# KadAMRN/Data_Free_Quantization

Hardware: AMD Instinct MI355X
Metric: weight-GB/s quantized (per-ch INT8 DFQ sweep) + top-1 delta, MobileNetV2 (higher is better)
Workload: dtype f32

## Files before the change

data_free_quantization_amd/csrc/dfq_common.h:

```cpp
#pragma once
#include <hip/hip_runtime.h>
#include <stdint.h>
#include <stdlib.h>
#include "dfq_hip.h"
#include "dfq_cle_plan.h"

namespace dfq {

__device__ __forceinline__ uint32_t enc_ord(float f) {
    uint32_t u = __float_as_uint(f);
    return (u & 0x80000000u) ? ~u : (u | 0x80000000u);
}
__device__ __forceinline__ float dec_ord(uint32_t e) {
    uint32_t u = (e & 0x80000000u) ? (e & 0x7fffffffu) : ~e;
    return __uint_as_float(u);
}

__device__ __forceinline__ float dpp_f(float v, int ctrl) {
    const int x = __float_as_int(v);
    switch (ctrl) {
        case 0xB1: return __int_as_float(__builtin_amdgcn_update_dpp(x, x, 0xB1, 0xF, 0xF, false));
        case 0x4E: return __int_as_float(__builtin_amdgcn_update_dpp(x, x, 0x4E, 0xF, 0xF, false));
        case 0x141: return __int_as_float(__builtin_amdgcn_update_dpp(x, x, 0x141, 0xF, 0xF, false));
        default: return __int_as_float(__builtin_amdgcn_update_dpp(x, x, 0x140, 0xF, 0xF, false));
// ... 331 lines not shown
__device__ inline float wave_full_sum(Get get, int64_t n, int threads, int lane, float* slots) {
    int64_t nt = 1;
    if (n >= 32768 && threads > 1) nt = ceil_div(n, (int64_t)32768) < threads ? ceil_div(n, (int64_t)32768) : threads;
    if (nt == 1) return wave_inner_sum(get, n, lane);
    const int64_t chunk = ceil_div(n, nt);
    for (int t = lane; t < threads; t += 64) slots[t] = 0.f;
    wave_lds_sync();
    for (int64_t t = 0; t < nt && t * chunk < n; ++t) {
        const int64_t b0 = t * chunk, len = (b0 + chunk < n ? b0 + chunk : n) - b0;
        const float s = wave_inner_sum([&](int64_t i) { return get(b0 + i); }, len, lane);
        if (lane == 0) slots[t] = s;
    }
    wave_lds_sync();
    float r = 0.f;
    if (lane == 0) r = aten_inner_sum([&](int64_t t) { return slots[t]; }, (int64_t)threads);
    wave_lds_sync();
    return __shfl(r, 0, 64);
}

#define DFQ_GLOBAL __attribute__((address_space(1)))
#define DFQ_LDS __attribute__((address_space(3)))
typedef float f32x4 __attribute__((ext_vector_type(4)));

__device__ __forceinline__ void st_coh(float* p, float v) {
    __hip_atomic_store(reinterpret_cast<uint32_t*>(p), __float_as_uint(v), __ATOMIC_RELAXED,
                       __HIP_MEMORY_SCOPE_AGENT);
}
__device__ __forceinline__ float ld_coh(const float* p) {
    return __uint_as_float(__hip_atomic_load(reinterpret_cast<const uint32_t*>(p), __ATOMIC_RELAXED,
                                             __HIP_MEMORY_SCOPE_AGENT));
}
__device__ __forceinline__ float ld_coh(const DFQ_GLOBAL float* p) {
    return __uint_as_float(__hip_atomic_load((const DFQ_GLOBAL uint32_t*)p, __ATOMIC_RELAXED,
                                             __HIP_MEMORY_SCOPE_AGENT));
}

__host__ __device__ inline bool aten_outer_col_is_cascade(int64_t R, int64_t F, int64_t c, int threads) {
    int64_t c0 = 0, c1 = F;
    if (R * F >= 32768 && threads > 1) {
        const int64_t nt = F < threads ? F : threads;
        const int64_t chunk = ceil_div(F, nt);
        c0 = c1 = -1;
        for (int64_t t = 0; t < nt; ++t) {
            int64_t b = t * chunk, e = b + chunk < F ? b + chunk : F;
            if (b >= F) break;
            b = b >= F ? b : b - b % 32;
            e = e >= F ? e : e - e % 32;
            if (b <= c && c < e) { c0 = b; c1 = e; break; }
        }
        if (c0 < 0) { c0 = 0; c1 = F; }
    }
    const int64_t w = c1 - c0;
    const int64_t g = w >= 8 ? 32 : 4;
    return (c - c0) < g * (w / g);
}

__host__ __device__ inline float aten_outer_col_sum(const float* a, int64_t R, int64_t F, int64_t c, int threads) {
    int64_t c0 = 0, c1 = F;
    if (R * F >= 32768 && threads > 1) {
        const int64_t nt = F < threads ? F : threads;
        const int64_t chunk = ceil_div(F, nt);
        c0 = c1 = -1;
        for (int64_t t = 0; t < nt; ++t) {
            int64_t b = t * chunk, e = b + chunk < F ? b + chunk : F;
            if (b >= F) break;
            b = b >= F ? b : b - b % 32;
            e = e >= F ? e : e - e % 32;
            if (b <= c && c < e) { c0 = b; c1 = e; break; }
        }
        if (c0 < 0) { c0 = 0; c1 = F; }
    }
    const int64_t w = c1 - c0;
    const int64_t g = w >= 8 ? 32 : 4;
    const bool cascade = (c - c0) < g * (w / g);
    auto get = [&](int64_t r) { return a[r * F + c]; };
    return cascade ? aten_cascade(get, R) : aten_row_sum(get, R);
}

}

namespace dfq {
void set_last_hip_error(hipError_t e);
void set_last_hip_error_text(const char* msg);
hipError_t stage_h2d(void* dst, const void* src, size_t bytes, hipStream_t s);
}
#define DFQ_HIP_CHECK(expr)                                   \
    do {                                                      \
        hipError_t _e = (expr);                               \
        if (_e != hipSuccess) {                               \
            dfq::set_last_hip_error(_e);                      \
            return DFQ_ERR_HIP;                               \
        }                                                     \
    } while (0)
#define DFQ_LAUNCH_CHECK()                                    \
    do {                                                      \
        hipError_t _e = hipGetLastError();                    \
        if (_e != hipSuccess) {                               \
            dfq::set_last_hip_error(_e);                      \
            return DFQ_ERR_HIP;                               \
        }                                                     \
    } while (0)
```

data_free_quantization_amd/csrc/dfq_lib.hip:

```cpp
#include "dfq_common.h"

#include <algorithm>
#include <cstring>
#include <mutex>
#include <vector>

namespace dfq {
static thread_local char g_last_hip[256] = "";
void set_last_hip_error(hipError_t e) {
    const char* msg = hipGetErrorString(e);
    size_t i = 0;
    for (; msg && msg[i] && i + 1 < sizeof(g_last_hip); ++i) g_last_hip[i] = msg[i];
    g_last_hip[i] = '\0';
}
void set_last_hip_error_text(const char* msg) {
    size_t i = 0;
    for (; msg && msg[i] && i + 1 < sizeof(g_last_hip); ++i) g_last_hip[i] = msg[i];
    g_last_hip[i] = '\0';
}

namespace {
struct StageSlot {
    void* host = nullptr;
    size_t cap = 0;
    hipEvent_t ev = nullptr;
    int device = -1;
    uint64_t last_use = 0;
};
constexpr size_t kStageMinBytes = 1 << 20;
constexpr size_t kStageMaxSlots = 32;
std::mutex g_stage_mu;
std::vector<StageSlot> g_stage;
uint64_t g_stage_tick = 0;
}

hipError_t stage_h2d(void* dst, const void* src, size_t bytes, hipStream_t s) {
    if (bytes == 0) return hipSuccess;
    int dev = 0;
    hipError_t e = hipStreamGetDevice(s, &dev);
    if (e != hipSuccess) return e;
    std::lock_guard<std::mutex> lock(g_stage_mu);
    StageSlot* slot = nullptr;
    StageSlot* oldest = nullptr;
    size_t on_dev = 0;
    for (auto& sl : g_stage) {
        if (sl.device != dev) continue;
        ++on_dev;
        if (sl.cap >= bytes && hipEventQuery(sl.ev) == hipSuccess &&
            (!slot || sl.cap < slot->cap)) slot = &sl;
        if (!oldest || sl.last_use < oldest->last_use) oldest = &sl;
    }
    if (!slot && on_dev >= kStageMaxSlots && oldest) {
        if ((e = hipEventSynchronize(oldest->ev)) != hipSuccess) return e;
        if (oldest->cap < bytes) {
            (void)hipHostFree(oldest->host);
            oldest->host = nullptr;
            oldest->cap = 0;
            size_t cap = std::max(bytes, kStageMinBytes);
            if ((e = hipHostMalloc(&oldest->host, cap, hipHostMallocDefault)) != hipSuccess) return e;
            oldest->cap = cap;
        }
        slot = oldest;
    }
    if (!slot) {
        StageSlot ns;
        ns.device = dev;
        ns.cap = std::max(bytes, kStageMinBytes);
        int cur = 0;
        if ((e = hipGetDevice(&cur)) != hipSuccess) return e;
        if (cur != dev && (e = hipSetDevice(dev)) != hipSuccess) return e;
        e = hipHostMalloc(&ns.host, ns.cap, hipHostMallocDefault);
        if (e == hipSuccess) e = hipEventCreateWithFlags(&ns.ev, hipEventDisableTiming);
        if (cur != dev) (void)hipSetDevice(cur);
        if (e != hipSuccess) {
            if (ns.host) (void)hipHostFree(ns.host);
            return e;
        }
        g_stage.push_back(ns);
        slot = &g_stage.back();
    }
    std::memcpy(slot->host, src, bytes);
    if ((e = hipMemcpyAsync(dst, slot->host, bytes, hipMemcpyHostToDevice, s)) != hipSuccess) return e;
    slot->last_use = ++g_stage_tick;
    return hipEventRecord(slot->ev, s);
}
}

namespace dfq {
static hipError_t stage_preload(size_t n) {
    int dev = 0;
    hipError_t e = hipGetDevice(&dev);
    if (e != hipSuccess) return e;
    std::lock_guard<std::mutex> lock(g_stage_mu);
    size_t on_dev = 0;
    for (const auto& sl : g_stage) on_dev += sl.device == dev ? 1 : 0;
    for (; on_dev < n && on_dev < kStageMaxSlots; ++on_dev) {
        StageSlot ns;
        ns.device = dev;
        ns.cap = kStageMinBytes;
        if ((e = hipHostMalloc(&ns.host, ns.cap, hipHostMallocDefault)) != hipSuccess) return e;
        if ((e = hipEventCreateWithFlags(&ns.ev, hipEventDisableTiming)) != hipSuccess) {
            (void)hipHostFree(ns.host);
            return e;
        }
        g_stage.push_back(ns);
    }
    return hipSuccess;
}
constexpr size_t kStagePreloadSlots = 8;

hipError_t preload_sweep();
hipError_t preload_transform();
hipError_t preload_cle();
hipError_t preload_stats();
hipError_t preload_clip();
hipError_t preload_mx();
}

extern "C" int dfq_preload(void) {
    DFQ_HIP_CHECK(dfq::preload_sweep());
    DFQ_HIP_CHECK(dfq::preload_transform());
    DFQ_HIP_CHECK(dfq::preload_cle());
    DFQ_HIP_CHECK(dfq::preload_stats());
    DFQ_HIP_CHECK(dfq::preload_clip());
    DFQ_HIP_CHECK(dfq::preload_mx());
    DFQ_HIP_CHECK(dfq::stage_preload(dfq::kStagePreloadSlots));
    return DFQ_OK;
}

extern "C" int dfq_abi_version(void) { return DFQ_ABI_VERSION; }

extern "C" const char* dfq_last_hip_error(void) { return dfq::g_last_hip; }

extern "C" const char* dfq_error_string(int code) {
    switch (code) {
        case DFQ_OK: return "ok";
        case DFQ_ERR_INVALID: return "invalid argument";
        case DFQ_ERR_HIP: return "HIP runtime error";
        case DFQ_ERR_UNSUPPORTED: return "unsupported request";
        case DFQ_ERR_NOMEM: return "out of memory";
        case DFQ_ERR_SHAPE: return "shape mismatch";
        case DFQ_ERR_WORKSPACE: return "workspace too small";
        default: return "unknown error";
    }
}
```

data_free_quantization_amd/csrc/dfq_transform.hip:

```cpp
#include "dfq_common.h"

#include <cstdlib>
#include <cstring>

#include <algorithm>
#include <chrono>
#include <cmath>
#include <mutex>
#include <new>
#include <string>
#include <vector>

namespace dfq {

static int blocks_for(int64_t n, int per_thread = 1) {
    const int64_t b = ceil_div(std::max<int64_t>(n, 1), (int64_t)kThreads * per_thread);
    return (int)std::min<int64_t>(b, 256 * 8);
}

__device__ __forceinline__ float bn_factor(float g, float v, float eps) {
    return g / sqrtf(v + eps);
}

__global__ void bn_fold_weight_kernel(float* __restrict__ w, const float* __restrict__ g,
                                      const float* __restrict__ v, float eps, int64_t rows, int64_t len) {
    const int64_t n = rows * len;
    for (int64_t i = (int64_t)blockIdx.x * blockDim.x + threadIdx.x; i < n; i += (int64_t)gridDim.x * blockDim.x) {
        const int64_t o = i / len;
        w[i] = w[i] * bn_factor(g[o], v[o], eps);
    }
}

__global__ void bn_fold_channel_kernel(float* __restrict__ bias, float* __restrict__ g, float* __restrict__ b,
                                       float* __restrict__ m, float* __restrict__ v, float* __restrict__ fake_w,
                                       float* __restrict__ fake_b, float eps, int64_t rows) {
    for (int64_t o = (int64_t)blockIdx.x * blockDim.x + threadIdx.x; o < rows; o += (int64_t)gridDim.x * blockDim.x) {
        const float go = g[o], bo = b[o], mo = m[o], vo = v[o];
        const float f = bn_factor(go, vo, eps);
        const float shift = bo - (go * mo) / sqrtf(vo + eps);
        bias[o] = bias[o] * f + shift;
        if (fake_w) fake_w[o] = fabsf(go);
        if (fake_b) fake_b[o] = bo;
        g[o] = 1.0f;
        v[o] = 1.0f;
        b[o] = 0.0f;
        m[o] = 0.0f;
    }
}

__global__ void clamp_kernel(float* __restrict__ w, int64_t n, float lo, float hi) {
    const int64_t n4 = n >> 2;
    float4* w4 = reinterpret_cast<float4*>(w);
    for (int64_t i = (int64_t)blockIdx.x * blockDim.x + threadIdx.x; i < n4; i += (int64_t)gridDim.x * blockDim.x) {
        float4 v = w4[i];
        v.x = fminf(fmaxf(v.x, lo), hi);
        v.y = fminf(fmaxf(v.y, lo), hi);
        v.z = fminf(fmaxf(v.z, lo), hi);
        v.w = fminf(fmaxf(v.w, lo), hi);
        w4[i] = v;
    }
    for (int64_t i = 4 * n4 + (int64_t)blockIdx.x * blockDim.x + threadIdx.x; i < n; i += (int64_t)gridDim.x * blockDim.x)
        w[i] = fminf(fmaxf(w[i], lo), hi);
}

__device__ __forceinline__ float absorb_c(float beta, float gamma, float n_sigma) {
    float c = beta - n_sigma * gamma;
    return (c < 0.0f) ? 0.0f : c;
}

__global__ void absorb_gemv_kernel(const float* __restrict__ w2, float* __restrict__ b2,
                                   const float* __restrict__ bn_w, const float* __restrict__ bn_b,
                                   int64_t o2, int64_t i2, int64_t khw2, int64_t o2g, float n_sigma) {
    const int lane = threadIdx.x & 63;
    const int64_t wave = (int64_t)blockIdx.x * (blockDim.x / 64) + (threadIdx.x >> 6);
    const int64_t nwaves = (int64_t)gridDim.x * (blockDim.x / 64);
    for (int64_t o = wave; o < o2; o += nwaves) {
        const int64_t g = o / o2g;
        const float* row = w2 + o * i2 * khw2;
        float acc = 0.f;
        for (int64_t i = lane; i < i2; i += 64) {
            float ssum = 0.f;
            for (int64_t k = 0; k < khw2; ++k) ssum += row[i * khw2 + k];
            const int64_t ch = g * i2 + i;
// ... 172 lines not shown
            const float x0 = (-b) / w;
            const float P0 = std_pdf(x0), C0 = std_cdf(x0);
            m = w * P0 + b * (1.0f - C0);
            const float B = ((b * b + w * w) + m * m) - (2.0f * m) * b;
            v = ((1.0f - C0) * B + (w * (b - 2.0f * m)) * P0) + (m * m) * C0;
        } else {
            const float x0 = (-b) / w, x6 = (6.0f - b) / w;
            const float P0 = std_pdf(x0), C0 = std_cdf(x0), P6 = std_pdf(x6), C6 = std_cdf(x6);
            m = (w * (P0 - P6) + b * (C6 - C0)) + 6.0f * (1.0f - C6);
            const float B = ((b * b + w * w) + m * m) - (2.0f * m) * b;
            const float d6 = 6.0f - m;
            v = ((((C6 - C0) * B + (w * -6.0f) * P6) + (w * (b - 2.0f * m)) * (P0 - P6)) + (m * m) * C0) +
                (d6 * d6) * (1.0f - C6);
        }
        if (accumulate) {
            m = mean[j] + m;
            v = var[j] + v;
        }
        mean[j] = m;
        var[j] = v;
    }
}

__global__ void act_minmax_kernel(const float* a, const float* w_in, int64_t n, int w_is_var, float eps, float nsig,
                                  float* out) {
    __shared__ float smin[4], smax[4];
    float vmin = INFINITY, vmax = -INFINITY;
    for (int64_t j = threadIdx.x; j < n; j += blockDim.x) {
        const float w = w_is_var ? sqrtf(w_in[j] + eps) : w_in[j];
        const float nw = nsig * w;
        vmin = fminf(vmin, a[j] - nw);
        vmax = fmaxf(vmax, a[j] + nw);
    }
    vmin = wave_min(vmin);
    vmax = wave_max(vmax);
    if ((threadIdx.x & 63) == 0) {
        smin[threadIdx.x >> 6] = vmin;
        smax[threadIdx.x >> 6] = vmax;
    }
    __syncthreads();
    if (threadIdx.x == 0) {
        for (int k = 1; k < (int)(blockDim.x / 64); ++k) {
            vmin = fminf(vmin, smin[k]);
            vmax = fmaxf(vmax, smax[k]);
        }
        out[0] = fminf(smin[0], vmin);
        out[1] = fmaxf(smax[0], vmax);
    }
}

__global__ void act_affine_kernel(const float* x, const float* w, const float* bias, int64_t o, int64_t i2,
                                  int64_t khw, int64_t og, float* out) {
    const int lane = threadIdx.x & 63;
    const int64_t wave = (int64_t)blockIdx.x * (blockDim.x / 64) + (threadIdx.x >> 6);
    const int64_t nwaves = (int64_t)gridDim.x * (blockDim.x / 64);
    for (int64_t r = wave; r < o; r += nwaves) {
        const int64_t g = r / og;
        float acc = 0.f;
        for (int64_t i = lane; i < i2; i += 64) {
            const float* p = w + (r * i2 + i) * khw;
            const float ws = khw == 1 ? p[0] : aten_inner_sum([&](int64_t k) { return p[k]; }, khw);
            acc += ws * x[g * i2 + i];
        }
        acc = wave_sum_f(acc);
        if (lane == 0) out[r] = bias ? acc + bias[r] : acc;
    }
}


struct BnFoldJob {
    float* w;
    float* bias;
    float* g;
    float* b;
    float* m;
    float* v;
    float* fake_w;
    float* fake_b;
    float eps;
    int32_t flags;
    int64_t rows, row_len;
    uint32_t* range_enc;
};
struct BnFoldChunk {
    int32_t job;
    int32_t pad;
    int64_t e0, e1;
};

__device__ __forceinline__ float fold_factor(const BnFoldJob& J, int64_t o) {
    const float go = ((const DFQ_GLOBAL float*)J.g)[o], ve = ((const DFQ_GLOBAL float*)J.v)[o] + J.eps;
    return (go == 1.0f && ve == 1.0f) ? 1.0f : go / sqrtf(ve);
}

__device__ __forceinline__ int64_t fold_row(const BnFoldJob& J, int64_t r0, int64_t base, float inv, int64_t i,
                                            int* rem_out) {
    const int li = (int)(i - base);
    const int len = (int)J.row_len;
    int q = (int)((float)li * inv);
    int rem = li - q * len;
    if (rem < 0) {
        --q;
        rem += len;
    } else if (rem >= len) {
        ++q;
        rem -= len;
    }
    *rem_out = rem;
    return r0 + q;
}

__device__ __forceinline__ float fold_one(const BnFoldJob& J, int64_t r0, int64_t base, float inv, int64_t i,
                                          float w) {
    int rem;
    const float f = fold_factor(J, fold_row(J, r0, base, inv, i, &rem));
    return f != 1.0f ? w * f : w;
}

__global__ void __launch_bounds__(kThreads)
bn_fold_weight_batch_kernel(const BnFoldJob* __restrict__ jobs, const BnFoldChunk* __restrict__ chunks,
                            int64_t nchunks) {
    __shared__ float smn[kThreads / kWave], smx[kThreads / kWave];
    for (int64_t c = blockIdx.x; c < nchunks; c += gridDim.x) {
        const BnFoldChunk ch = chunks[c];
        const BnFoldJob J = jobs[ch.job];
        const int64_t r0 = ch.e0 / J.row_len, base = r0 * J.row_len;
        const float inv = 1.0f / (float)J.row_len;
        float a = INFINITY, b = -INFINITY;
        const int64_t n = ch.e1 - ch.e0;
        int64_t done = 0;
        int ident = 1;
        for (int64_t r = r0 + threadIdx.x; r <= (ch.e1 - 1) / J.row_len; r += blockDim.x)
            ident &= fold_factor(J, r) == 1.0f;
        ident = __syncthreads_and(ident);
        if (ident && (reinterpret_cast<uintptr_t>(J.w + ch.e0) & 15) == 0) {
            const DFQ_GLOBAL f32x4* w4 = (const DFQ_GLOBAL f32x4*)(J.w + ch.e0);
            const int64_t n4 = n >> 2;
            for (int64_t k = threadIdx.x; k < n4; k += 4 * (int64_t)blockDim.x) {
                f32x4 v[4];
#pragma unroll
                for (int u = 0; u < 4; ++u)
                    if (k + u * (int64_t)blockDim.x < n4) v[u] = w4[k + u * blockDim.x];
#pragma unroll
                for (int u = 0; u < 4; ++u)
                    if (k + u * (int64_t)blockDim.x < n4) {
                        a = fminf(a, fminf(fminf(v[u].x, v[u].y), fminf(v[u].z, v[u].w)));
                        b = fmaxf(b, fmaxf(fmaxf(v[u].x, v[u].y), fmaxf(v[u].z, v[u].w)));
                    }
            }
            done = 4 * n4;
        } else if ((reinterpret_cast<uintptr_t>(J.w + ch.e0) & 15) == 0) {
            DFQ_GLOBAL f32x4* w4 = (DFQ_GLOBAL f32x4*)(J.w + ch.e0);
            const int64_t n4 = n >> 2;
            for (int64_t k = threadIdx.x; k < n4; k += blockDim.x) {
                const f32x4 v = w4[k];
                const int64_t i = ch.e0 + 4 * k;
                f32x4 o;
                int rem;
                const float f = fold_factor(J, fold_row(J, r0, base, inv, i, &rem));
                if (rem + 3 < (int)J.row_len) {
                    o.x = f != 1.0f ? v.x * f : v.x;
                    o.y = f != 1.0f ? v.y * f : v.y;
                    o.z = f != 1.0f ? v.z * f : v.z;
                    o.w = f != 1.0f ? v.w * f : v.w;
                } else {
                    o.x = f != 1.0f ? v.x * f : v.x;
                    o.y = fold_one(J, r0, base, inv, i + 1, v.y);
                    o.z = fold_one(J, r0, base, inv, i + 2, v.z);
                    o.w = fold_one(J, r0, base, inv, i + 3, v.w);
                }
                if (__float_as_uint(o.x) != __float_as_uint(v.x) || __float_as_uint(o.y) != __float_as_uint(v.y) ||
                    __float_as_uint(o.z) != __float_as_uint(v.z) || __float_as_uint(o.w) != __float_as_uint(v.w))
                    w4[k] = o;
                a = fminf(a, fminf(fminf(o.x, o.y), fminf(o.z, o.w)));
                b = fmaxf(b, fmaxf(fmaxf(o.x, o.y), fmaxf(o.z, o.w)));
            }
            done = 4 * n4;
        }
        DFQ_GLOBAL float* wg = (DFQ_GLOBAL float*)J.w;
        for (int64_t k = done + threadIdx.x; k < n; k += blockDim.x) {
            const int64_t i = ch.e0 + k;
            const float v = wg[i];
            const float o = fold_one(J, r0, base, inv, i, v);
            if (__float_as_uint(o) != __float_as_uint(v)) wg[i] = o;
            a = fminf(a, o);
            b = fmaxf(b, o);
        }
        if (J.range_enc) {
            a = wave_min(a);
            b = wave_max(b);
            const int lane = threadIdx.x & (kWave - 1), wv = threadIdx.x >> 6;
            if (lane == 0) {
                smn[wv] = a;
                smx[wv] = b;
            }
            __syncthreads();
            if (threadIdx.x == 0) {
                for (int k = 1; k < kThreads / kWave; ++k) {
                    a = fminf(a, smn[k]);
                    b = fmaxf(b, smx[k]);
                }
                atomicMax(&J.range_enc[0], ~enc_ord(a));
                atomicMax(&J.range_enc[1], enc_ord(b));
            }
            __syncthreads();
        }
    }
}

__global__ void bn_fold_channel_batch_kernel(const BnFoldJob* __restrict__ jobs, int32_t njobs) {
    for (int32_t j = blockIdx.x; j < njobs; j += gridDim.x) {
        const BnFoldJob J = jobs[j];
        typedef DFQ_GLOBAL float* G;
        const G g = (G)J.g, b = (G)J.b, m = (G)J.m, v = (G)J.v, bias = (G)J.bias, fw = (G)J.fake_w, fb = (G)J.fake_b;
        for (int64_t o = threadIdx.x; o < J.rows; o += blockDim.x) {
            const float go = g[o], bo = b[o], mo = m[o], vo = v[o];
            const float f = bn_factor(go, vo, J.eps);
            const float shift = bo - (go * mo) / sqrtf(vo + J.eps);
            const float b0 = (J.flags & DFQ_BN_FOLD_ZERO_BIAS) ? 0.0f : bias[o];
            bias[o] = b0 * f + shift;
            if (J.fake_w) fw[o] = fabsf(go);
            if (J.fake_b) fb[o] = bo;
            g[o] = 1.0f;
            v[o] = 1.0f;
            b[o] = 0.0f;
            m[o] = 0.0f;
        }
    }
}

__device__ __forceinline__ float qdq_nan(float x, const QParams& p, float& q) {
    const float y = qdq(x, p, q);
    return x != x ? x : y;
}

__global__ void __launch_bounds__(kThreads)
fq_given_kernel(const float* __restrict__ x, float* __restrict__ y, int64_t n, int bits, int sym, int flags,
                const float* __restrict__ min_dev, const float* __restrict__ max_dev,
                const uint32_t* __restrict__ range_enc, double gmin, double gmax, int vec4) {
    if (min_dev) gmin = (double)min_dev[0];
    if (max_dev) gmax = (double)max_dev[0];
    if (range_enc) {
        gmin = (double)dec_ord(~range_enc[0]);
        gmax = (double)dec_ord(range_enc[1]);
    }
    const QParams p = make_qparams((float)gmin, (float)gmax, bits, sym != 0, flags | DFQ_GIVEN_RANGE, gmin, gmax);
    const int64_t stride = (int64_t)gridDim.x * blockDim.x;
    float q;
    if (vec4) {
        const int64_t n4 = n >> 2;
        for (int64_t i = (int64_t)blockIdx.x * blockDim.x + threadIdx.x; i < n4; i += stride) {
            const float4 v = reinterpret_cast<const float4*>(x)[i];
            float4 o;
            o.x = qdq_nan(v.x, p, q);
            o.y = qdq_nan(v.y, p, q);
            o.z = qdq_nan(v.z, p, q);
            o.w = qdq_nan(v.w, p, q);
            reinterpret_cast<float4*>(y)[i] = o;
        }
    } else {
        for (int64_t i = (int64_t)blockIdx.x * blockDim.x + threadIdx.x; i < n; i += stride)
            y[i] = qdq_nan(x[i], p, q);
    }
}

constexpr int64_t kFqSmall = 16384;

__global__ void __launch_bounds__(kThreads)
fq_tensor_small_kernel(const float* __restrict__ x, float* __restrict__ y, int64_t n, int bits, int sym, int flags) {
    __shared__ float smn[kThreads / kWave], smx[kThreads / kWave];
    float a = INFINITY, b = -INFINITY;
    for (int64_t i = threadIdx.x; i < n; i += kThreads) {
        const float v = x[i];
        a = fminf(a, v);
        b = fmaxf(b, v);
    }
    a = wave_min(a);
    b = wave_max(b);
    const int lane = threadIdx.x & (kWave - 1), w = threadIdx.x >> 6;
    if (lane == 0) {
        smn[w] = a;
        smx[w] = b;
    }
    __syncthreads();
    for (int k = 0; k < kThreads / kWave; ++k) {
        a = k ? fminf(a, smn[k]) : smn[0];
        b = k ? fmaxf(b, smx[k]) : smx[0];
    }
// ... 640 lines not shown
    for (int32_t k = 0; k < n_ops; ++k) {
        const dfq_bc_op& op = ops[k];
        int rc = DFQ_OK;
        if (op.kind == DFQ_BC_OP_EXPECT) {
            dfq::BcLayerJob J{};
            const int32_t used = dfq::bc_layer_group(ops, n_ops, k, J);
            if (used > 0) {
                const int64_t pb = J.fake_b ? std::min<int64_t>(ceil_div(J.F, (int64_t)4), 2048) : 0;
                hipLaunchKernelGGL(dfq::bc_layer_kernel, dim3((int)(J.apply_blocks + pb)), dim3(kThreads), 0,
                                   static_cast<hipStream_t>(stream), J);
                const hipError_t e = hipGetLastError();
                if (e != hipSuccess) {
                    dfq::set_last_hip_error(e);
                    return fail(k, DFQ_ERR_HIP);
                }
                k += used - 1;
                continue;
            }
        }
        if (op.kind == DFQ_BC_OP_COPY) {
            CopyBatch b{};
            int cnt = 0;
            int64_t most = 0;
            int32_t j = k;
            for (; j < n_ops && ops[j].kind == DFQ_BC_OP_COPY && cnt < kCopyBatch; ++j) {
                if (ops[j].n == 0) continue;
                b.src[cnt] = ops[j].a;
                b.dst[cnt] = ops[j].out;
                b.n[cnt] = ops[j].n;
                most = std::max(most, ops[j].n);
                ++cnt;
            }
            if (cnt > 0) {
                hipLaunchKernelGGL(copy_batch_kernel, dim3(blocks_for(most), cnt), dim3(256), 0,
                                   static_cast<hipStream_t>(stream), b);
                const hipError_t e = hipGetLastError();
                if (e != hipSuccess) {
                    dfq::set_last_hip_error(e);
                    return fail(k, DFQ_ERR_HIP);
                }
            }
            k = j - 1;
            continue;
        }
        if (op.kind == DFQ_BC_OP_EXPECT)
            rc = dfq_bc_expect(op.a, op.b, op.n, op.flag & 1, (op.flag >> 1) & 1, op.out, stream);
        else if (op.kind == DFQ_BC_OP_APPLY)
            rc = dfq_bc_apply(op.a, op.n, op.i2, op.b, op.f, op.out, op.out2, nullptr, stream);
        else
            rc = dfq_bc_propagate(op.a, op.n, op.out, op.f, op.flag, stream);
        if (rc != DFQ_OK) return fail(k, rc);
    }
    return DFQ_OK;
}

extern "C" int dfq_act_moments(const float* w, const float* b, int64_t n, int32_t kind, int32_t sqrt_w, float eps,
                               int32_t accumulate, float* mean, float* var, void* stream) {
    if (!w || !b || !mean || !var || n < 0 || kind < 0 || kind > 2) return DFQ_ERR_INVALID;
    if (n == 0) return DFQ_OK;
    hipLaunchKernelGGL(act_moments_kernel, dim3(blocks_for(n)), dim3(kThreads), 0, static_cast<hipStream_t>(stream), w,
                       b, n, (int)kind, (int)sqrt_w, eps, (int)accumulate, mean, var);
    DFQ_LAUNCH_CHECK();
    return DFQ_OK;
}

extern "C" int dfq_act_minmax(const float* a, const float* w, int64_t n, int32_t w_is_var, float eps, float nsig,
                              float* out2, void* stream) {
    if (!a || !w || !out2 || n <= 0) return DFQ_ERR_INVALID;
    hipLaunchKernelGGL(act_minmax_kernel, dim3(1), dim3(kThreads), 0, static_cast<hipStream_t>(stream), a, w, n,
                       (int)w_is_var, eps, nsig, out2);
    DFQ_LAUNCH_CHECK();
    return DFQ_OK;
}

extern "C" int dfq_act_affine(const float* x, const float* w, const float* bias, int64_t o, int64_t i2, int64_t khw,
                              int64_t groups, float* out, void* stream) {
    if (!x || !w || !out || o <= 0 || i2 <= 0 || khw <= 0 || groups <= 0 || o % groups) return DFQ_ERR_INVALID;
    hipLaunchKernelGGL(act_affine_kernel, dim3((int)std::min<int64_t>(ceil_div(o, (int64_t)4), 2048)), dim3(kThreads),
                       0, static_cast<hipStream_t>(stream), x, w, bias, o, i2, khw, o / groups, out);
    DFQ_LAUNCH_CHECK();
    return DFQ_OK;
}

static int64_t bn_fold_span(const dfq_bn_fold_desc* d, int32_t n) {
    int64_t total = 0;
    for (int32_t j = 0; j < n; ++j) total += d[j].rows * d[j].row_len;
    return std::min<int64_t>(std::max<int64_t>(8192, ceil_div(total, (int64_t)16384 * 8192) * 8192), 1 << 20);
}

static int bn_fold_tables(const dfq_bn_fold_desc* d, int32_t n, std::vector<BnFoldJob>& jobs,
                          std::vector<BnFoldChunk>& chunks) {
    const int64_t span = bn_fold_span(d, n);
    {
        std::vector<const float*> ws(n);
        for (int32_t j = 0; j < n; ++j) ws[j] = d[j].w;
        std::sort(ws.begin(), ws.end());
        if (std::adjacent_find(ws.begin(), ws.end()) != ws.end()) return DFQ_ERR_INVALID;
    }
    jobs.resize(n);
    for (int32_t j = 0; j < n; ++j) {
        const dfq_bn_fold_desc& x = d[j];
        if (!x.w || !x.bias || !x.bn_w || !x.bn_b || !x.bn_mean || !x.bn_var || x.rows < 0 || x.row_len < 0)
            return DFQ_ERR_INVALID;
        if (x.row_len > (int64_t(1) << 22)) return DFQ_ERR_UNSUPPORTED;
        jobs[j] = BnFoldJob{x.w, x.bias, x.bn_w, x.bn_b, x.bn_mean, x.bn_var, x.fake_w, x.fake_b, x.eps, x.flags, x.rows,
                            x.row_len, x.range_enc};
        const int64_t ne = x.rows * x.row_len;
        for (int64_t e = 0; e < ne; e += span) chunks.push_back(BnFoldChunk{j, 0, e, std::min<int64_t>(e + span, ne)});
    }
    return DFQ_OK;
}

static int64_t round256(int64_t b) { return ceil_div(b, (int64_t)256) * 256; }

extern "C" int64_t dfq_bn_fold_ws_bytes(const dfq_bn_fold_desc* d, int32_t n) {
    if (n < 0 || (n > 0 && !d)) return -1;
    int64_t nchunks = 0;
    for (int32_t j = 0; j < n; ++j)
        if (d[j].rows < 0 || d[j].row_len < 0) return -1;
    const int64_t span = bn_fold_span(d, n);
    for (int32_t j = 0; j < n; ++j) nchunks += ceil_div(d[j].rows * d[j].row_len, span);
    return round256((int64_t)sizeof(BnFoldJob) * n) + round256((int64_t)sizeof(BnFoldChunk) * nchunks);
}

extern "C" int dfq_bn_fold_batch(const dfq_bn_fold_desc* d, int32_t n, void* ws, int64_t ws_bytes, void* stream) {
    if (n < 0 || (n > 0 && !d)) return DFQ_ERR_INVALID;
    if (n == 0) return DFQ_OK;
    std::vector<BnFoldJob> jobs;
    std::vector<BnFoldChunk> chunks;
    const int rc = bn_fold_tables(d, n, jobs, chunks);
    if (rc != DFQ_OK) return rc;
    const int64_t jb = round256((int64_t)sizeof(BnFoldJob) * n);
    const int64_t need = jb + round256((int64_t)sizeof(BnFoldChunk) * (int64_t)chunks.size());
    if (ws && (ws_bytes < need || reinterpret_cast<uintptr_t>(ws) % 256 != 0)) return DFQ_ERR_INVALID;
    hipStream_t s = static_cast<hipStream_t>(stream);
    void* own = nullptr;
    if (!ws) {
        DFQ_HIP_CHECK(hipMalloc(&own, need));
        ws = own;
    }
    char* base = static_cast<char*>(ws);
    BnFoldJob* dj = reinterpret_cast<BnFoldJob*>(base);
    BnFoldChunk* dc = reinterpret_cast<BnFoldChunk*>(base + jb);
    std::vector<char> blob(need, 0);
    std::memcpy(blob.data(), jobs.data(), sizeof(BnFoldJob) * n);
    if (!chunks.empty()) std::memcpy(blob.data() + jb, chunks.data(), sizeof(BnFoldChunk) * chunks.size());
    hipError_t e = own ? hipMemcpyAsync(base, blob.data(), need, hipMemcpyHostToDevice, s)
                       : stage_h2d(base, blob.data(), need, s);
    std::vector<uint32_t*> rp;
    for (int32_t j = 0; j < n; ++j)
        if (d[j].range_enc) rp.push_back(d[j].range_enc);
    std::sort(rp.begin(), rp.end());
    for (size_t k = 0; k < rp.size() && e == hipSuccess;) {
        size_t m = k + 1;
        while (m < rp.size() && rp[m] == rp[m - 1] + 2) ++m;
        e = hipMemsetAsync(rp[k], 0, sizeof(uint32_t) * 2 * (m - k), s);
        k = m;
    }
    if (e == hipSuccess && !chunks.empty()) {
        hipLaunchKernelGGL(bn_fold_weight_batch_kernel, dim3((int)std::min<size_t>(chunks.size(), 4096)),
                           dim3(kThreads), 0, s, dj, dc, (int64_t)chunks.size());
        e = hipGetLastError();
    }
    if (e == hipSuccess) {
        hipLaunchKernelGGL(bn_fold_channel_batch_kernel, dim3(std::min(n, 2048)), dim3(kThreads), 0, s, dj, n);
        e = hipGetLastError();
    }
    if (e == hipSuccess && own) e = hipStreamSynchronize(s);
    if (own) (void)hipFree(own);
    if (e != hipSuccess) {
        set_last_hip_error(e);
        return DFQ_ERR_HIP;
    }
    return DFQ_OK;
}

extern "C" int dfq_chunk_range(const float* x, int64_t rows, int64_t row_len, float* rowbuf, float* out2,
                               void* stream) {
    if (!x || !rowbuf || !out2 || rows < 1) return DFQ_ERR_INVALID;
    if (row_len < 1) return DFQ_ERR_SHAPE;
    hipStream_t s = static_cast<hipStream_t>(stream);
    const int grid = (int)std::min<int64_t>(rows, 4096);
    hipLaunchKernelGGL(chunk_row_range_kernel, dim3(grid), dim3(kThreads), 0, s, x, rows, row_len, rowbuf,
                       rowbuf + rows);
    DFQ_LAUNCH_CHECK();
    hipLaunchKernelGGL(chunk_mean_kernel, dim3(1), dim3(kWave), 0, s, rowbuf, rowbuf + rows, rows, out2);
    DFQ_LAUNCH_CHECK();
    return DFQ_OK;
}

extern "C" int dfq_act_observe(const float* x, int64_t rows, int64_t row_len, uint32_t* words, float* running_min,
                               float* running_max, int32_t update_stat, int32_t training, double momentum,
                               float* out2, void* stream) {
    if (!x || !words || !running_min || !running_max || !out2 || rows < 1) return DFQ_ERR_INVALID;
    if (row_len < 1) return DFQ_ERR_SHAPE;
    hipStream_t s = static_cast<hipStream_t>(stream);
    const int64_t slices = std::max<int64_t>(1, std::min<int64_t>(ceil_div(row_len, (int64_t)16384),
                                                                  ceil_div((int64_t)1024, rows)));
    const int grid = (int)std::min<int64_t>(rows * slices, 8192);
    hipLaunchKernelGGL(observe_rows_kernel, dim3(grid), dim3(kThreads), 0, s, x, rows, row_len, slices, words);
    DFQ_LAUNCH_CHECK();
    hipLaunchKernelGGL(observe_finish_kernel, dim3(1), dim3(kWave), 0, s, words, rows, running_min, running_max,
                       update_stat, training, (float)(1.0 - momentum), (float)momentum, out2);
    DFQ_LAUNCH_CHECK();
    return DFQ_OK;
}

extern "C" int dfq_range(const float* x, int64_t n, uint32_t* range_enc, void* stream) {
    if (n < 1 || !x || !range_enc) return DFQ_ERR_INVALID;
    hipStream_t s = static_cast<hipStream_t>(stream);
    DFQ_HIP_CHECK(hipMemsetAsync(range_enc, 0, 2 * sizeof(uint32_t), s));
    const int grid = (int)std::min<int64_t>(ceil_div(n, (int64_t)kThreads * 8), 2048);
    hipLaunchKernelGGL(range_enc_kernel, dim3(std::max(grid, 1)), dim3(kThreads), 0, s, x, n, range_enc);
    DFQ_LAUNCH_CHECK();
    return DFQ_OK;
}

extern "C" int dfq_fake_quant_tensor(const float* x, float* y, int64_t n, int32_t bits, int32_t symmetric,
                                     int32_t flags, uint32_t* words, void* stream) {
    if (n < 1 || !x || !y || bits < 2 || bits > 16) return DFQ_ERR_INVALID;
    if (flags & ~(DFQ_SCALE_F32)) return DFQ_ERR_INVALID;
    hipStream_t s = static_cast<hipStream_t>(stream);
    if (n <= kFqSmall) {
        hipLaunchKernelGGL(fq_tensor_small_kernel, dim3(1), dim3(kThreads), 0, s, x, y, n, bits, symmetric, flags);
        DFQ_LAUNCH_CHECK();
        return DFQ_OK;
    }
    if (!words) return DFQ_ERR_INVALID;
    const int grid = (int)std::min<int64_t>(ceil_div(n, (int64_t)kThreads * 8), 2048);
    hipLaunchKernelGGL(fq_tensor_range_kernel, dim3(std::max(grid, 1)), dim3(kThreads), 0, s, x, n, words);
    DFQ_LAUNCH_CHECK();
    const int vec4 = (n % 4 == 0) && (reinterpret_cast<uintptr_t>(x) % 16 == 0) &&
                     (reinterpret_cast<uintptr_t>(y) % 16 == 0);
    const int64_t work = vec4 ? n / 4 : n;
    const int g2 = (int)std::min<int64_t>(ceil_div(work, (int64_t)kThreads * 4), 16384);
    hipLaunchKernelGGL(fq_given_kernel, dim3(std::max(g2, 1)), dim3(kThreads), 0, s, x, y, n, bits, symmetric, flags,
                       nullptr, nullptr, static_cast<const uint32_t*>(words + 4), 0.0, 0.0, vec4);
    DFQ_LAUNCH_CHECK();
    return DFQ_OK;
}

extern "C" int dfq_fake_quant_given(const float* x, float* y, int64_t n, int32_t bits, int32_t symmetric,
                                    int32_t flags, const float* min_dev, const float* max_dev,
                                    const uint32_t* range_enc, double given_min, double given_max, void* stream) {
// ... 22 lines not shown
```

Measured before the change: 1894.

## Split BN-fold chunks into per-wave units and upload tables via a kernel

```diff
diff --git a/data_free_quantization_amd/csrc/dfq_common.h b/data_free_quantization_amd/csrc/dfq_common.h
--- a/data_free_quantization_amd/csrc/dfq_common.h
+++ b/data_free_quantization_amd/csrc/dfq_common.h
@@ -437,7 +437,9 @@
 namespace dfq {
 void set_last_hip_error(hipError_t e);
 void set_last_hip_error_text(const char* msg);
-hipError_t stage_h2d(void* dst, const void* src, size_t bytes, hipStream_t s);
+typedef hipError_t (*StageSend)(void* dst, const void* pinned, size_t bytes, hipStream_t s, void* arg);
+hipError_t stage_h2d(void* dst, const void* src, size_t bytes, hipStream_t s, StageSend send = nullptr,
+                     void* arg = nullptr);
 }
 #define DFQ_HIP_CHECK(expr)                                   \
     do {                                                      \
diff --git a/data_free_quantization_amd/csrc/dfq_fold_plan.h b/data_free_quantization_amd/csrc/dfq_fold_plan.h
--- /dev/null
+++ b/data_free_quantization_amd/csrc/dfq_fold_plan.h
@@ -0,0 +1,41 @@
+#pragma once
+#include <algorithm>
+
+#include "dfq_cle_plan.h"
+
+namespace dfq {
+
+struct BnFoldChunk {
+    int32_t job;
+    int32_t pad;
+    int64_t e0, e1;
+};
+
+inline int64_t bn_fold_span(int64_t total) {
+    return std::min<int64_t>(std::max<int64_t>(8192, ceil_div(total, (int64_t)16384 * 8192) * 8192), 1 << 20);
+}
+
+#ifndef DFQ_FOLD_UNIT_MAX
+#define DFQ_FOLD_UNIT_MAX 16384
+#endif
+constexpr int64_t kFoldUnitMin = 2048, kFoldUnitMax = DFQ_FOLD_UNIT_MAX;
+static_assert(kFoldUnitMax >= kFoldUnitMin && (kFoldUnitMax & (kFoldUnitMax - 1)) == 0, "a power of two");
+inline int64_t bn_fold_unit(int64_t total) {
+    int64_t u = kFoldUnitMin;
+    while (u < kFoldUnitMax && ceil_div(total, u) > 65536) u *= 2;
+    return u;
+}
+inline int64_t bn_fold_units_per_chunk(int64_t span, int64_t unit) { return ceil_div(span, unit); }
+
+DFQ_HOST_DEVICE inline bool bn_fold_unit_piece(int64_t e0, int64_t e1, int64_t p, int64_t unit, int64_t* s0,
+                                               int64_t* s1) {
+    *s0 = e0 + p * unit;
+    *s1 = *s0 + unit < e1 ? *s0 + unit : e1;
+    return *s0 < e1;
+}
+
+inline void bn_fold_chunks_of(int32_t job, int64_t ne, int64_t span, std::vector<BnFoldChunk>& chunks) {
+    for (int64_t e = 0; e < ne; e += span) chunks.push_back(BnFoldChunk{job, 0, e, std::min<int64_t>(e + span, ne)});
+}
+
+}
diff --git a/data_free_quantization_amd/csrc/dfq_lib.hip b/data_free_quantization_amd/csrc/dfq_lib.hip
--- a/data_free_quantization_amd/csrc/dfq_lib.hip
+++ b/data_free_quantization_amd/csrc/dfq_lib.hip
@@ -34,7 +34,7 @@
 uint64_t g_stage_tick = 0;
 }
 
-hipError_t stage_h2d(void* dst, const void* src, size_t bytes, hipStream_t s) {
+hipError_t stage_h2d(void* dst, const void* src, size_t bytes, hipStream_t s, StageSend send, void* arg) {
     if (bytes == 0) return hipSuccess;
     int dev = 0;
     hipError_t e = hipStreamGetDevice(s, &dev);
@@ -80,7 +80,8 @@
         slot = &g_stage.back();
     }
     std::memcpy(slot->host, src, bytes);
-    if ((e = hipMemcpyAsync(dst, slot->host, bytes, hipMemcpyHostToDevice, s)) != hipSuccess) return e;
+    e = send ? send(dst, slot->host, bytes, s, arg) : hipMemcpyAsync(dst, slot->host, bytes, hipMemcpyHostToDevice, s);
+    if (e != hipSuccess) return e;
     slot->last_use = ++g_stage_tick;
     return hipEventRecord(slot->ev, s);
 }
diff --git a/data_free_quantization_amd/csrc/dfq_transform.hip b/data_free_quantization_amd/csrc/dfq_transform.hip
--- a/data_free_quantization_amd/csrc/dfq_transform.hip
+++ b/data_free_quantization_amd/csrc/dfq_transform.hip
@@ -1,4 +1,5 @@
 #include "dfq_common.h"
+#include "dfq_fold_plan.h"
 
 #include <cstdlib>
 #include <cstring>
@@ -337,12 +338,6 @@
     int64_t rows, row_len;
     uint32_t* range_enc;
 };
-struct BnFoldChunk {
-    int32_t job;
-    int32_t pad;
-    int64_t e0, e1;
-};
-
 __device__ __forceinline__ float fold_factor(const BnFoldJob& J, int64_t o) {
     const float go = ((const DFQ_GLOBAL float*)J.g)[o], ve = ((const DFQ_GLOBAL float*)J.v)[o] + J.eps;
     return (go == 1.0f && ve == 1.0f) ? 1.0f : go / sqrtf(ve);
@@ -372,44 +367,110 @@
     return f != 1.0f ? w * f : w;
 }
 
+#ifndef DFQ_RANGE_LOADS
+#define DFQ_RANGE_LOADS 8
+#endif
+#ifndef DFQ_RANGE_NT
+#define DFQ_RANGE_NT 1
+#endif
+constexpr int kRangeLoads = DFQ_RANGE_LOADS;
+__device__ __forceinline__ f32x4 range_ld(const DFQ_GLOBAL f32x4* p) {
+    if constexpr (DFQ_RANGE_NT) return __builtin_nontemporal_load(p);
+    else return *p;
+}
+__device__ __forceinline__ void range_acc(const f32x4& v, float& lo, float& hi) {
+    lo = fminf(lo, fminf(fminf(v.x, v.y), fminf(v.z, v.w)));
+    hi = fmaxf(hi, fmaxf(fmaxf(v.x, v.y), fmaxf(v.z, v.w)));
+}
+__device__ __forceinline__ void wave_range_stream(const DFQ_GLOBAL f32x4* p, int n4, int lane, float& lo, float& hi) {
+    constexpr int U = kRangeLoads;
+    const int trips = n4 / (U * kWave);
+    if (trips > 0) {
+        const DFQ_GLOBAL f32x4* q = p + lane;
+        f32x4 va[U], vb[U];
+        auto load = [&](f32x4* v) {
+#pragma unroll
+            for (int u = 0; u < U; ++u) v[u] = range_ld(q + u * kWave);
+            q += U * kWave;
+            __builtin_amdgcn_sched_barrier(0);
+        };
+        auto reduce = [&](const f32x4* v) {
+#pragma unroll
+            for (int u = 0; u < U; ++u) range_acc(v[u], lo, hi);
+        };
+        load(va);
+        int t = 1;
+        for (; t + 1 < trips; t += 2) {
+            load(vb);
+            reduce(va);
+            load(va);
+            reduce(vb);
+        }
+        if (t < trips) {
+            load(vb);
+            reduce(va);
+            reduce(vb);
+        } else {
+            reduce(va);
+        }
+    }
+    const int k0 = trips * U * kWave + lane;
+    f32x4 v[U];
+#pragma unroll
+    for (int u = 0; u < U; ++u)
+        if (k0 + u * kWave < n4) v[u] = range_ld(p + k0 + u * kWave);
+#pragma unroll
+    for (int u = 0; u < U; ++u)
+        if (k0 + u * kWave < n4) range_acc(v[u], lo, hi);
+}
+
+#ifndef DFQ_FOLD_UPLOAD_KERNEL
+#define DFQ_FOLD_UPLOAD_KERNEL 1
+#endif
+__global__ void __launch_bounds__(kThreads)
+bn_fold_upload_kernel(const uint4* __restrict__ src, uint4* __restrict__ dst, int64_t n16, int32_t njobs) {
+    const int64_t t = (int64_t)blockIdx.x * kThreads + threadIdx.x, nt = (int64_t)gridDim.x * kThreads;
+    constexpr int64_t kJobWords = sizeof(BnFoldJob) / 16, kRangeWord = offsetof(BnFoldJob, range_enc) / 16;
+    static_assert(sizeof(BnFoldJob) % 16 == 0 && offsetof(BnFoldJob, range_enc) % 16 == 8, "range_enc: a word's upper half");
+    for (int64_t k = t; k < n16; k += nt) {
+        const uint4 w = src[k];
+        dst[k] = w;
+        if (k < njobs * kJobWords && k % kJobWords == kRangeWord) {
+            DFQ_GLOBAL uint32_t* re = (DFQ_GLOBAL uint32_t*)(((uint64_t)w.w << 32) | w.z);
+            if (re) re[0] = re[1] = 0u;
+        }
+    }
+}
+
 __global__ void __launch_bounds__(kThreads)
 bn_fold_weight_batch_kernel(const BnFoldJob* __restrict__ jobs, const BnFoldChunk* __restrict__ chunks,
-                            int64_t nchunks) {
-    __shared__ float smn[kThreads / kWave], smx[kThreads / kWave];
-    for (int64_t c = blockIdx.x; c < nchunks; c += gridDim.x) {
+                            int64_t nunits, int32_t upc, int32_t unit) {
+    const int lane = threadIdx.x & (kWave - 1);
+    const int64_t wave0 = (int64_t)blockIdx.x * (kThreads / kWave) + wave_uniform(threadIdx.x >> 6);
+    const int64_t nwaves = (int64_t)gridDim.x * (kThreads / kWave);
+    for (int64_t u = wave0; u < nunits; u += nwaves) {
+        const int64_t c = u / upc;
         const BnFoldChunk ch = chunks[c];
+        int64_t s0, s1;
+        if (!bn_fold_unit_piece(ch.e0, ch.e1, u - c * upc, unit, &s0, &s1)) continue;
         const BnFoldJob J = jobs[ch.job];
-        const int64_t r0 = ch.e0 / J.row_len, base = r0 * J.row_len;
+        const int64_t r0 = s0 / J.row_len, r1 = (s1 - 1) / J.row_len, base = r0 * J.row_len;
         const float inv = 1.0f / (float)J.row_len;
         float a = INFINITY, b = -INFINITY;
-        const int64_t n = ch.e1 - ch.e0;
-        int64_t done = 0;
+        const int n = (int)(s1 - s0);
+        int done = 0;
+        const bool vec = (reinterpret_cast<uintptr_t>(J.w + s0) & 15) == 0;
         int ident = 1;
-        for (int64_t r = r0 + threadIdx.x; r <= (ch.e1 - 1) / J.row_len; r += blockDim.x)
-            ident &= fold_factor(J, r) == 1.0f;
-        ident = __syncthreads_and(ident);
-        if (ident && (reinterpret_cast<uintptr_t>(J.w + ch.e0) & 15) == 0) {
-            const DFQ_GLOBAL f32x4* w4 = (const DFQ_GLOBAL f32x4*)(J.w + ch.e0);
-            const int64_t n4 = n >> 2;
-            for (int64_t k = threadIdx.x; k < n4; k += 4 * (int64_t)blockDim.x) {
-                f32x4 v[4];
-#pragma unroll
-                for (int u = 0; u < 4; ++u)
-                    if (k + u * (int64_t)blockDim.x < n4) v[u] = w4[k + u * blockDim.x];
-#pragma unroll
-                for (int u = 0; u < 4; ++u)
-                    if (k + u * (int64_t)blockDim.x < n4) {
-                        a = fminf(a, fminf(fminf(v[u].x, v[u].y), fminf(v[u].z, v[u].w)));
-                        b = fmaxf(b, fmaxf(fmaxf(v[u].x, v[u].y), fmaxf(v[u].z, v[u].w)));
-                    }
-            }
-            done = 4 * n4;
-        } else if ((reinterpret_cast<uintptr_t>(J.w + ch.e0) & 15) == 0) {
-            DFQ_GLOBAL f32x4* w4 = (DFQ_GLOBAL f32x4*)(J.w + ch.e0);
-            const int64_t n4 = n >> 2;
-            for (int64_t k = threadIdx.x; k < n4; k += blockDim.x) {
+        for (int64_t r = r0 + lane; r <= r1; r += kWave) ident &= fold_factor(J, r) == 1.0f;
+        if (vec && __all(ident)) {
+            wave_range_stream((const DFQ_GLOBAL f32x4*)(J.w + s0), n >> 2, lane, a, b);
+            done = n & ~3;
+        } else if (vec) {
+            DFQ_GLOBAL f32x4* w4 = (DFQ_GLOBAL f32x4*)(J.w + s0);
+            const int n4 = n >> 2;
+            for (int k = lane; k < n4; k += kWave) {
                 const f32x4 v = w4[k];
-                const int64_t i = ch.e0 + 4 * k;
+                const int64_t i = s0 + 4 * k;
                 f32x4 o;
                 int rem;
                 const float f = fold_factor(J, fold_row(J, r0, base, inv, i, &rem));
@@ -433,8 +494,8 @@
             done = 4 * n4;
         }
         DFQ_GLOBAL float* wg = (DFQ_GLOBAL float*)J.w;
-        for (int64_t k = done + threadIdx.x; k < n; k += blockDim.x) {
-            const int64_t i = ch.e0 + k;
+        for (int k = done + lane; k < n; k += kWave) {
+            const int64_t i = s0 + k;
             const float v = wg[i];
             const float o = fold_one(J, r0, base, inv, i, v);
             if (__float_as_uint(o) != __float_as_uint(v)) wg[i] = o;
@@ -444,21 +505,11 @@
         if (J.range_enc) {
             a = wave_min(a);
             b = wave_max(b);
-            const int lane = threadIdx.x & (kWave - 1), wv = threadIdx.x >> 6;
             if (lane == 0) {
-                smn[wv] = a;
-                smx[wv] = b;
+                DFQ_GLOBAL uint32_t* re = (DFQ_GLOBAL uint32_t*)J.range_enc;
+                __hip_atomic_fetch_max(&re[0], ~enc_ord(a), __ATOMIC_RELAXED, __HIP_MEMORY_SCOPE_AGENT);
+                __hip_atomic_fetch_max(&re[1], enc_ord(b), __ATOMIC_RELAXED, __HIP_MEMORY_SCOPE_AGENT);
             }
-            __syncthreads();
-            if (threadIdx.x == 0) {
-                for (int k = 1; k < kThreads / kWave; ++k) {
-                    a = fminf(a, smn[k]);
-                    b = fmaxf(b, smx[k]);
-                }
-                atomicMax(&J.range_enc[0], ~enc_ord(a));
-                atomicMax(&J.range_enc[1], enc_ord(b));
-            }
-            __syncthreads();
         }
     }
 }
@@ -1265,15 +1316,15 @@
     return DFQ_OK;
 }
 
-static int64_t bn_fold_span(const dfq_bn_fold_desc* d, int32_t n) {
+static int64_t bn_fold_total(const dfq_bn_fold_desc* d, int32_t n) {
     int64_t total = 0;
     for (int32_t j = 0; j < n; ++j) total += d[j].rows * d[j].row_len;
-    return std::min<int64_t>(std::max<int64_t>(8192, ceil_div(total, (int64_t)16384 * 8192) * 8192), 1 << 20);
+    return total;
 }
 
 static int bn_fold_tables(const dfq_bn_fold_desc* d, int32_t n, std::vector<BnFoldJob>& jobs,
                           std::vector<BnFoldChunk>& chunks) {
-    const int64_t span = bn_fold_span(d, n);
+    const int64_t span = bn_fold_span(bn_fold_total(d, n));
     {
         std::vector<const float*> ws(n);
         for (int32_t j = 0; j < n; ++j) ws[j] = d[j].w;
@@ -1288,8 +1339,7 @@
         if (x.row_len > (int64_t(1) << 22)) return DFQ_ERR_UNSUPPORTED;
         jobs[j] = BnFoldJob{x.w, x.bias, x.bn_w, x.bn_b, x.bn_mean, x.bn_var, x.fake_w, x.fake_b, x.eps, x.flags, x.rows,
                             x.row_len, x.range_enc};
-        const int64_t ne = x.rows * x.row_len;
-        for (int64_t e = 0; e < ne; e += span) chunks.push_back(BnFoldChunk{j, 0, e, std::min<int64_t>(e + span, ne)});
+        bn_fold_chunks_of(j, x.rows * x.row_len, span, chunks);
     }
     return DFQ_OK;
 }
@@ -1301,7 +1351,7 @@
     int64_t nchunks = 0;
     for (int32_t j = 0; j < n; ++j)
         if (d[j].rows < 0 || d[j].row_len < 0) return -1;
-    const int64_t span = bn_fold_span(d, n);
+    const int64_t span = bn_fold_span(bn_fold_total(d, n));
     for (int32_t j = 0; j < n; ++j) nchunks += ceil_div(d[j].rows * d[j].row_len, span);
     return round256((int64_t)sizeof(BnFoldJob) * n) + round256((int64_t)sizeof(BnFoldChunk) * nchunks);
 }
@@ -1328,21 +1378,41 @@
     std::vector<char> blob(need, 0);
     std::memcpy(blob.data(), jobs.data(), sizeof(BnFoldJob) * n);
     if (!chunks.empty()) std::memcpy(blob.data() + jb, chunks.data(), sizeof(BnFoldChunk) * chunks.size());
-    hipError_t e = own ? hipMemcpyAsync(base, blob.data(), need, hipMemcpyHostToDevice, s)
-                       : stage_h2d(base, blob.data(), need, s);
-    std::vector<uint32_t*> rp;
-    for (int32_t j = 0; j < n; ++j)
-        if (d[j].range_enc) rp.push_back(d[j].range_enc);
-    std::sort(rp.begin(), rp.end());
-    for (size_t k = 0; k < rp.size() && e == hipSuccess;) {
-        size_t m = k + 1;
-        while (m < rp.size() && rp[m] == rp[m - 1] + 2) ++m;
-        e = hipMemsetAsync(rp[k], 0, sizeof(uint32_t) * 2 * (m - k), s);
-        k = m;
+    const bool by_kernel = DFQ_FOLD_UPLOAD_KERNEL && !own;
+    hipError_t e;
+    if (by_kernel) {
+        int32_t njobs = n;
+        e = stage_h2d(base, blob.data(), need, s,
+                      [](void* dst, const void* pinned, size_t bytes, hipStream_t st, void* arg) {
+                          const int64_t n16 = (int64_t)(bytes / 16);
+                          hipLaunchKernelGGL(bn_fold_upload_kernel,
+                                             dim3((int)std::min<int64_t>(ceil_div(n16, (int64_t)kThreads), 2048)),
+                                             dim3(kThreads), 0, st, static_cast<const uint4*>(pinned),
+                                             static_cast<uint4*>(dst), n16, *static_cast<int32_t*>(arg));
+                          return hipGetLastError();
+                      },
+                      &njobs);
+    } else {
+        e = own ? hipMemcpyAsync(base, blob.data(), need, hipMemcpyHostToDevice, s)
+                : stage_h2d(base, blob.data(), need, s);
+        std::vector<uint32_t*> rp;
+        for (int32_t j = 0; j < n; ++j)
+            if (d[j].range_enc) rp.push_back(d[j].range_enc);
+        std::sort(rp.begin(), rp.end());
+        for (size_t k = 0; k < rp.size() && e == hipSuccess;) {
+            size_t m = k + 1;
+            while (m < rp.size() && rp[m] == rp[m - 1] + 2) ++m;
+            e = hipMemsetAsync(rp[k], 0, sizeof(uint32_t) * 2 * (m - k), s);
+            k = m;
+        }
     }
     if (e == hipSuccess && !chunks.empty()) {
-        hipLaunchKernelGGL(bn_fold_weight_batch_kernel, dim3((int)std::min<size_t>(chunks.size(), 4096)),
-                           dim3(kThreads), 0, s, dj, dc, (int64_t)chunks.size());
+        const int64_t total = bn_fold_total(d, n), unit = bn_fold_unit(total);
+        const int64_t upc = bn_fold_units_per_chunk(bn_fold_span(total), unit);
+        const int64_t nunits = (int64_t)chunks.size() * upc;
+        hipLaunchKernelGGL(bn_fold_weight_batch_kernel,
+                           dim3((int)std::min<int64_t>(ceil_div(nunits, (int64_t)(kThreads / kWave)), 16384)),
+                           dim3(kThreads), 0, s, dj, dc, nunits, (int32_t)upc, (int32_t)unit);
         e = hipGetLastError();
     }
     if (e == hipSuccess) {
```

New measurement: 1920 (median of 3 runs). Within noise of the previous version (+1.4%).
